# tomstrident/GAN-based-Video-Style-Transfer

Hardware: AMD Instinct MI355X
Metric: frames/sec: CycleGAN train step (G+D+flow-warp loss) 256x256 (higher is better)
Workload: dtype fp32; 1 GPU; C2: CycleGANCon optimize_parameters, resnet_9blocks G + basic PatchGAN D, ngf=ndf=64, 256x256, B_local=4, pool_size=50, flow-warp temporal loss; global_batch=4, height=256, width=256, parallelism=dp1

## Files before the change

### gan-based-video-style-transfer_amd/_lib.py

```python
import ctypes
import glob
import os
import subprocess

import torch

PKG = os.path.dirname(os.path.abspath(__file__))
REPO = os.path.dirname(PKG)
BUILD = os.path.join(PKG, "_build")
LIB_PATH = os.path.join(BUILD, "libvst_hip.so")
LIB_PATH = os.environ.get("VST_LIB_VARIANT") or LIB_PATH
CSRC = os.path.join(PKG, "csrc")
HIPCC = os.environ.get("HIPCC", "/opt/rocm/bin/hipcc")
ARCH = "gfx950"

_lib = None


def source_stamp():
    import hashlib
    h = hashlib.sha1()
    for f in sorted(glob.glob(os.path.join(CSRC, "*"))) + [os.path.join(REPO, "include", "vst_hip.h")]:
        if f.endswith((".hip", ".h")):
            h.update(os.path.basename(f).encode())
# ... 39 lines not shown
    "vst_instnorm_ws_bytes": (SZ, [I, I, I]),
    "vst_instnorm_stats": (I, [P, P, P, I, I, I, F, P]),
    "vst_instnorm_act_fwd": (I, [P, P, P, P, I, I, I, I, F, P]),
    "vst_instnorm_act_bwd": (I, [P, P, P, P, P, P, I, I, I, I, F, I, P]),
    "vst_instnorm_act_bwd_planes": (I, [P, P, P, P, P, P, I, I, I, I, F, I, P, L, P]),
    "vst_conv2d_wgrad_nhwc_ok": (I, [I, I, I, I, I, I, I, I, I, I, I, I]),
    "vst_conv2d_wgrad_nhwc_ws_bytes": (SZ, [I, I, I, I, I, I, I, I, I, I, I, I]),
    "vst_conv2d_wgrad_nhwc": (I, [P, P, P, P, SZ, I, I, I, I, I, I, I, I, I, I, I, I, I, I, L, L, I, I, P]),
    "vst_conv2d_wgrad_nhwc_f32_ok": (I, [I, I, I, I, I, I, I, I, I, I, I, I]),
    "vst_conv2d_wgrad_nhwc_f32_ws_bytes": (SZ, [I, I, I, I, I, I, I, I, I, I, I, I]),
    "vst_conv2d_wgrad_nhwc_f32": (I, [P, P, P, P, SZ, I, I, I, I, I, I, I, I, I, I, I, I, I, I, L, L, I, I, P]),
    "vst_conv2d_wgrad_pre": (I, [P, P, P, P, P, P, SZ, I, I, I, I, I, I, I, I, I, I, I, I, I, I, L, L, I, I, P]),
    "vst_instnorm_act_fwd_cp": (I, [P, P, P, P, P, I, I, I, I, I, F, I, I, I, P]),
    "vst_instnorm_act_fwd_planes": (I, [P, P, P, P, P, I, I, I, I, I, F, I, I, I, P]),
    "vst_cp_ld": (L, [L]),
    "vst_conv2d_fwd_co": (I, [P, P, P, P, P, I, I, I, I, I, I, I, I, I, I, I, F, I, I, P]),
    "vst_conv2d_fwd_co_ws_bytes": (SZ, [I, I, I, I, I, I, I, I, I, I, I]),
    "vst_conv2d_fwd_co_ws": (I, [P, P, P, P, P, I, I, I, I, I, I, I, I, I, I, I, F, I, I, P, SZ, P]),
    "vst_tapfold_planes": (I, [P, P, L, I, I, I, I, I, I, I, P]),
    "vst_conv2d_fwd_ws_bytes": (SZ, [I, I, I, I, I, I, I, I, I, I]),
    "vst_conv2d_fwd_ws": (I, [P, P, P, P, P, I, I, I, I, I, I, I, I, I, I, I, F, I, P, P, P, SZ, P]),
    "vst_c4_dgrad_frame": (I, [P, P, P, I, I, I, I, I, I, P]),
    "vst_conv_plan_fwd_tail": (I, [I, I, I, I, I, I, I, I, I, I, P]),
    "vst_act_bwd": (I, [P, P, P, L, I, F, P]),
    "vst_warp_fwd": (I, [P, P, P, I, I, I, I, I, P]),
    "vst_warp_bwd_input": (I, [P, P, P, I, I, I, I, I, P]),
    "vst_fbcheck": (I, [P, P, P, I, I, I, P]),
    "vst_loss_part_floats": (I, [L]),
    "vst_loss_temporal": (I, [P, P, P, P, P, P, I, I, I, I, I, F, P]),
    "vst_loss_temporal_bwd": (I, [P, P, P, P, P, P, P, I, I, I, I, I, F, P]),
    "vst_loss_l1": (I, [P, P, P, P, L, I, I, F, P]),
    "vst_loss_l1_bwd": (I, [P, P, P, P, L, I, I, F, P]),
    "vst_loss_mse_const": (I, [P, F, P, P, L, I, I, F, P]),
    "vst_loss_mse_const_bwd": (I, [P, F, P, P, L, I, I, F, P]),
    "vst_finish_sum": (I, [P, I, P, D, P]),
    "vst_adam_step": (I, [P, P, P, P, L, F, F, F, F, I, P]),
    "vst_axpby": (I, [P, P, L, F, F, P]),
    "vst_warp_masked_fwd": (I, [P, P, P, I, I, I, I, I, P]),
    "vst_warp_masked_bwd_input": (I, [P, P, P, I, I, I, I, I, P]),
    "vst_warp_bwd_det_ws_bytes": (SZ, [I, I, I]),
    "vst_warp_bwd_input_det": (I, [P, P, P, P, SZ, I, I, I, I, I, I, I, I, P]),
    "vst_temporal_sqdiff_part_floats": (I, [I, I, I, I]),
    "vst_temporal_sqdiff_fwd": (I, [P, P, P, P, P, P, P, P, I, I, I, I, I, F, F, P]),
    "vst_temporal_sqdiff_bwd": (I, [P, P, P, P, P, P, P, P, P, I, I, I, I, I, F, F, P]),
    "vst_resize_bilinear": (I, [P, P, P, I, I, I, I, I, I, P]),
    "vst_instnorm_affine_fwd": (I, [P, P, P, P, P, F, P, P, I, I, I, I, F, P]),
# ... 180 lines not shown
```

### gan-based-video-style-transfer_amd/csrc/common.h

```cpp
#pragma once
#include <hip/hip_runtime.h>
#include <stdint.h>
#include <stdio.h>
#include <string.h>

#include "../../include/vst_hip.h"

typedef float f32x16 __attribute__((ext_vector_type(16)));
typedef float f32x4v __attribute__((ext_vector_type(4)));

namespace vst {

void set_error(const char* fmt, ...);

inline int check_launch(const char* what) {
  hipError_t e = hipGetLastError();
  if (e != hipSuccess) {
    set_error("%s: %s", what, hipGetErrorString(e));
    return VST_EHIP;
  }
  return VST_OK;
}

#define VST_NUM_CUS 256
// ... 101 lines not shown
int bf_fprop_launch(const float* x, const void* wsplit, long wps, const float* bias, float* y, int N,
                    int H, int W, int C, int Ho, int Wo, int Cop, int R, int S, int st, int padh, int padw,
                    int reflect, int act, float slope, int math, int kind, hipStream_t s,
                    double* part = nullptr, float* tws = nullptr, size_t tws_floats = 0, const float* addend = nullptr,
                    int oph = 0);
bool tap64_ok(int Cx, int R, int W, int math);
int tap64_launch(const float* x, const void* wsplit, long wps, const float* bias, float* y, int N, int H, int W,
                 int pad, int reflect, int act, float slope, int math, hipStream_t s);
bool c4_direct_ok(int C, int Cop, int R, int S, int st, int Ho, int Wo, int math);
int c4_direct_launch(const float* x, const void* wsplit, long wps, const float* bias, float* y, int N, int H, int W,
                     int Ho, int Wo, int R, int S, int pad, int reflect, int act, float slope, int math, double* part,
                     hipStream_t s);
bool bf_dgrad_refl1_ok(int N, int H, int W, int Cy, int Cx, int math);
size_t bf_dgrad_refl1_ws_floats(int N, int H, int W, int Cy, int Cx, int math);
size_t bf_dgrad_refl1_slabs(int N, int H, int W, int Cy, int Cx, int math, BorderSlabs* b);
int bf_dgrad_refl1_launch(const float* dy, const void* wsplit, long wps, const float* addend, float* dx, int N, int H,
                          int W, int Cy, int Cx, int math, hipStream_t s, float* ws, size_t ws_floats, bool add_border);
bool bf_dgrad_refl1_inb_ok(int N, int H, int W, int Cy, int Cx, int math);
int bf_dgrad_refl1_inb_slices(int H, int W);
int bf_dgrad_refl1_inb_launch(const float* dy, const void* wsplit, long wps, const float* addend, float* dx, int N,
                              int H, int W, int Cy, int Cx, int math, hipStream_t s, float* ws, size_t ws_floats,
                              const float* z, const float* st, double* part, int act, float slope,
                              const __bf16* apl = nullptr, long pps = 0);
size_t bf_fprop_ws_floats(long M, int Cop, int C, int R, int S, int math);
int bf_tail_ks(long M, int Cop, int m_split, int nk);
void bf_split_plan(long M, int Cop, int C, int R, int S, int math, int kind, int* m_first, int* ks_out);
void bf_plan(long M, int Cop, int math, int kind, int* kind_out, int* m_split_out, int* tail_out);
void bf_nhwc_to_planes(const float* x, void* y, long P, int Cs, int np, hipStream_t s, int row_in = 0,
                       int row_out = 0);
void bf_wgrad_launch(const float* xt, const void* dyp, float* slab, int N, int H, int W, int Cx, int Ho,
                     int Wo, int Cyp, int S, int pad, int st, int Mw, int chunk, int nsplit, int kind, int math,
                     hipStream_t s);
void bf_wgrad_geom(int kind, int math, int* bm, int* bn, int* bk, int* slots);
bool bf_wgrad_nhwc_ok(int kind, int Wo, int Cx, int Cyp);
void bf_wgrad_nhwc_launch(const float* x, const void* dy, long pps, bool bf32, float* slab, int N, int H, int W,
                          int Cx, int Ho, int Wo, int Cyp, int S, int pad, int st, int reflect, int Mw, int chunk,
                          int nsplit, int kind, hipStream_t s, float* dwd = nullptr, int dco = 0, int dacc = 0);

void rk_tile_geom(int kind, int math, int* bm, int* bn, int* bk, int* slots);
void rk_nhwc_to_cp(const float* x, float* y, long P, int Cs, int pack, hipStream_t s);
void rk_nhwc_to_cp_pad(const float* x, float* y, int N, int H, int W, int Cs, int pad, int reflect,
                       int phase, int pack, hipStream_t s, int extra = 0);
void rk_wgrad_launch(const float* xt, const float* dyt, float* slab, int N, int H, int W, int Cx,
                     int Ho, int Wo, int Cyp, int S, int pad, int st, int Mw, int chunk,
                     int nsplit, int kind, int math, hipStream_t s);
void rk_tconv_launch(const float* in, const float* wp, const float* bias, const float* addend,
// ... 29 lines not shown
```

### gan-based-video-style-transfer_amd/csrc/conv.hip

```cpp
#include "common.h"

namespace vst {

constexpr int BK = 32;

template <int BM, int BN, int WM, int WN>
struct Tile {
  static constexpr int NW = (BM / WM) * (BN / WN);
  static constexpr int NT = 64 * NW;
  static constexpr int LDA = BM + 4;
  static constexpr int LDB = BN + 4;
  static constexpr int WAVES_N = BN / WN;
  static constexpr int MI = WM / 32;
  static constexpr int NI = WN / 32;
  static constexpr int A_ELEMS = BK * LDA;
  static constexpr int B_ELEMS = BK * LDB;
  static constexpr int STAGE = A_ELEMS + B_ELEMS;
  static_assert(NW == 4 || NW == 8, "4 or 8 waves per block");
  static_assert(WM % 32 == 0 && WN % 32 == 0, "32x32 MFMA blocks");
};

template <int BM, int BN, int WM, int WN, class Hook>
__device__ __forceinline__ void mma_stage(const float* __restrict__ As, const float* __restrict__ Bs,
                                          f32x16 (&acc)[WM / 32][WN / 32], int wm0, int wn0, int lane,
// ... 867 lines not shown
  return bf_fprop_ws_floats((long)N * Ho * Wo, Cop, Cx, R, S, math) * sizeof(float);
}

extern "C" int vst_conv2d_fwd_ws(const float* x, const float* wp, const void* wsplit, const float* bias, float* y,
                                 int N, int H, int W, int Cx, int Cop, int R, int S, int stride, int pad, int pad_mode,
                                 int act, float slope, int math, double* part, int* nsplit, float* ws,
                                 size_t ws_bytes, void* stream) {
  return conv_fwd_impl(x, wp, wsplit, bias, y, N, H, W, Cx, Cop, R, S, stride, pad, pad, pad_mode, act, slope,
                       math, (hipStream_t)stream, part, nsplit, ws, ws_bytes);
}

extern "C" int vst_conv_plan_fwd_tail(int N, int H, int W, int Cx, int Cop, int R, int S, int stride, int pad,
                                      int math, int* ksplit) {
  VST_REQUIRE(ksplit, "conv_plan_fwd_tail: null");
  *ksplit = 0;
  const size_t b = vst_conv2d_fwd_ws_bytes(N, H, W, Cx, Cop, R, S, stride, pad, math);
  if (b) {
    const int Ho = (H + 2 * pad - R) / stride + 1, Wo = (W + 2 * pad - S) / stride + 1;
    int mf;
    bf_split_plan((long)N * Ho * Wo, Cop, Cx, R, S, math, -1, &mf, ksplit);
  }
  return VST_OK;
}

extern "C" int vst_conv2d_fwd_hwp(const float* x, const float* wp, const void* wsplit, const float* bias, float* y,
                                  int N, int H, int W, int Cx, int Cop, int R, int S, int stride, int pad_h, int pad_w,
                                  int pad_mode, int act, float slope, int math, void* stream) {
  return conv_fwd_impl(x, wp, wsplit, bias, y, N, H, W, Cx, Cop, R, S, stride, pad_h, pad_w, pad_mode, act, slope,
                       math, (hipStream_t)stream);
}

extern "C" int vst_conv2d_fwd_hw(const float* x, const float* wp, const void* wsplit, const float* bias,
                                 float* y, int N, int H, int W, int Cx, int Cop, int R, int S, int stride,
                                 int pad_h, int pad_w, int act, float slope, int math, void* stream) {
  return conv_fwd_impl(x, wp, wsplit, bias, y, N, H, W, Cx, Cop, R, S, stride, pad_h, pad_w, VST_PAD_ZERO, act,
                       slope, math, (hipStream_t)stream);
}

extern "C" size_t vst_conv2d_fwd_hw_ws_bytes(int N, int H, int W, int Cx, int Cop, int R, int S, int stride, int pad_h,
                                             int pad_w, int math) {
  if (N <= 0 || H <= 0 || W <= 0 || R <= 0 || S <= 0 || stride <= 0 || Cx % 8 || Cop == 4) return 0;
  const int Ho = (H + 2 * pad_h - R) / stride + 1, Wo = (W + 2 * pad_w - S) / stride + 1;
  if (Ho <= 0 || Wo <= 0 || g_tile_override[0] >= 0) return 0;
  return bf_fprop_ws_floats((long)N * Ho * Wo, Cop, Cx, R, S, math) * sizeof(float);
}

// ... 472 lines not shown
```

### gan-based-video-style-transfer_amd/csrc/conv_bf.hip

```cpp
#include <type_traits>

#include "common.h"

#ifndef VST_BF_X6K3
#define VST_BF_X6K3 0
#endif
#ifndef VST_BF_MINB
#define VST_BF_MINB 1
#endif
#ifndef VST_BF_X6_256
#define VST_BF_X6_256 1
#endif
#ifndef VST_BF_KSLICE
#define VST_BF_KSLICE 1
#endif
#ifndef VST_BF_TAIL_KIND
#define VST_BF_TAIL_KIND 8
#endif
#ifndef VST_BF_TAIL
#define VST_BF_TAIL 1
#endif
#ifndef VST_BF_SCHED
#define VST_BF_SCHED 1
#endif
#ifndef VST_BF_PRIO
// ... 390 lines not shown
    if (!SA) {
      prep(P ^ 1);
      store_stage<T>(nxt, ra[P ^ 1], rbv[P ^ 1], rb, kq, !dmab.active, !dmab.a_active);
    }
    mma16<T>(mid, hi, acc);
    mma16<T>(hi, mid, acc);
    if (VST_M16_SCHED) sched16<2 * NM, RA ? 0 : NR, 0, SA ? 0 : 2, SA ? 0 : NW>();
    __builtin_amdgcn_sched_barrier(0);
    __syncthreads();
    read_plane16<T>(mid, nxt, 1, wm0, wn0, lane);
    mma16<T>(hi, hi, acc);
    mma16<T>(lo, hi, acc);
    mma16<T>(hi, lo, acc);
    if (VST_M16_SCHED) sched16<3 * NM, NR, 0, 0, 0>();
  };
  int kt = 0;
  for (; kt + 1 < nk; kt += 2) {
    step(kt, std::integral_constant<int, 0>());
    step(kt + 1, std::integral_constant<int, 1>());
  }
  if (kt < nk) step(kt, std::integral_constant<int, 0>());
}

template <int MI, int NI>
__device__ __forceinline__ void zero_acc4(f32x4v (&acc)[MI][NI]) {
#pragma unroll
  for (int i = 0; i < MI; ++i)
#pragma unroll
    for (int j = 0; j < NI; ++j) acc[i][j] = f32x4v{0.f, 0.f, 0.f, 0.f};
}

template <int MI, int NI>
__device__ __forceinline__ void zero_acc(f32x16 (&acc)[MI][NI]) {
#pragma unroll
  for (int i = 0; i < MI; ++i)
#pragma unroll
    for (int j = 0; j < NI; ++j)
#pragma unroll
      for (int r = 0; r < 16; ++r) acc[i][j][r] = 0.f;
}

__device__ __forceinline__ int remap_mtile(int bx, int nx) {
  if ((nx & 7) != 0) return bx;
  return (bx & 7) * (nx >> 3) + (bx >> 3);
}

// ... 204 lines not shown
  __syncthreads();
  if (t < 192) {
    const int v = t >> 6, cc = t & 63, nn = blockIdx.z * 64 + cc;
    if (nn >= C) return;
    double acc = 0.0;
    if (v < 2)
      for (int q = 0; q < 16; ++q) acc += red[v][q][cc];
    inb.part[(((long)n * inb.ns + first_slice + blockIdx.x) * C + nn) * 3 + v] = acc;
  }
}

__device__ __forceinline__ int phase_row(int mm, int oph, int Ho, int Wo) {
  const bool full = oph > 4;
  const int q = full ? oph - 5 : oph - 1, a = q >> 1, b = q & 1;
  const int hw = Ho * Wo, n = mm / hw, rem = mm - n * hw, ph = rem / Wo, pw = rem - ph * Wo;
  const int H = full ? Ho - 1 : Ho - a, W = full ? Wo - 1 : Wo - b;
  const int i = ph - a, j = pw - b;
  if (i < 0 || j < 0 || i >= H || j >= W) return -1;
  return (n * 2 * H + 2 * i + a) * 2 * W + 2 * j + b;
}

__device__ __attribute__((aligned(256))) float g_zero_page[64];

template <class T, bool KSL, int REFL, bool SPLIT, bool APRE = false>
__device__ __forceinline__ void conv_fprop_bf_body(
    int bid, const float* __restrict__ x, const __bf16* __restrict__ ws, long wps, const float* __restrict__ bias,
    float* __restrict__ y, int H, int W, int C, int Ho, int Wo, int Cop, int S, int st, int padh,
    int padw, int reflect, int act, float slope, int M, int Ktot, int m_base, double* __restrict__ part,
    int spk, float* __restrict__ slab, const float* __restrict__ addend, int oph,
    InbArgs inb = InbArgs{}, const __bf16* __restrict__ apl = nullptr, long pps = 0) {
  static_assert(!SPLIT || KSL, "split-K needs the channel-slice-major K walk");
  static_assert(REFL < 4 || (SPLIT && KSL), "border rows run as split-K slabs");
  __shared__ __attribute__((aligned(16))) char smem[2 * T::STAGE];
  constexpr int A_LD = T::A_LD, B_LD = T::B_LD, RPP = T::RPP, NP = T::NP;
  const int t = threadIdx.x, lane = t & 63, wave = t >> 6;
  int mt_, nt_;
  const int Mt_ = (M - m_base + T::BM - 1) / T::BM, Nt_ = (Cop + T::BN - 1) / T::BN;
  const int zs = SPLIT ? bid / (Mt_ * Nt_) : 0;
  tile_of(SPLIT ? bid - zs * Mt_ * Nt_ : bid, Mt_, Nt_, mt_, nt_);
  const int m0 = m_base + mt_ * T::BM, n0 = nt_ * T::BN;
  const int kq = t % T::KC, rb = t / T::KC;
  const float* zp = g_zero_page;

  constexpr bool C4 = REFL == 3;
  const int seg = REFL != 5 ? 0 : (m0 < Ho ? 0 : (m0 < 2 * Ho ? 1 : (m0 < 2 * Ho + Wo ? 2 : 3)));
  const int Sx = REFL != 5 ? S : (seg < 2 ? 3 : 1);
  int hb[A_LD], wb[A_LD], pb[A_LD], aoff[A_LD], aoff2[C4 ? A_LD : 1];
#pragma unroll
  for (int j = 0; j < A_LD; ++j) {
    const int m = m0 + rb + RPP * j;
    const int mm = m < M ? m : 0;
    if constexpr (REFL == 5) {
      const int L = seg < 2 ? W + 2 : H;
      const int r = mm - (seg == 0 ? 0 : (seg == 1 ? Ho : (seg == 2 ? 2 * Ho : 2 * Ho + Wo)));
      const int n = r / L, k = r - n * L;
      const bool live = (unsigned)r < (unsigned)(st * L);
// ... 184 lines not shown
      ts = go ? (w1 ? 0 : ts1) : ts;
      tr = go ? (w2 ? 0 : tr1) : tr;
      ksb = go ? ksb + (w2 ? T::BK : 0) : ksb;
      tap_rows(tr, ts);
      return;
    }
    if (!go) return;
    kcur += T::BK;
    kc += T::BK;
    if (kc >= C) {
      do {
        kc -= C;
        if (++ks == S) { ks = 0; ++kr; }
      } while (kc >= C);
      tap_rows(kr, ks);
    }
  };

  auto prep = [](int) __attribute__((always_inline)) {};
  const int wm0 = (wave / T::WAVES_N) * T::WM, wn0 = (wave % T::WAVES_N) * T::WN;
  if constexpr (T::M16) {
    f32x4v acc[T::MI16][T::NI16];
    zero_acc4(acc);
    if constexpr (GLDS)
      main_loop16<T>(smem, nk, acc, ra, rbv, rb, kq, load_all, adv, prep, DmaB<decltype(dma_b), GLDS_A>{dma_b});
    else
      main_loop16<T>(smem, nk, acc, ra, rbv, rb, kq, load_all, adv, prep, NoDma{});
    if constexpr (SPLIT) {
      float* sl = slab + (long)zs * (M - m_base) * Cop;
#pragma unroll
      for (int i = 0; i < T::MI16; ++i)
#pragma unroll
        for (int j = 0; j < T::NI16; ++j) {
          const int n = n0 + wn0 + 16 * j + (lane & 15);
#pragma unroll
          for (int r = 0; r < 4; ++r) {
            const int mm = m0 + wm0 + 16 * i + 4 * (lane >> 4) + r;
            if (n < Cop && mm < M) sl[(long)(mm - m_base) * Cop + n] = acc[i][j][r];
          }
        }
      return;
    }
    constexpr bool LFIT = T::BM * (T::BN + 16) * 4 <= 2 * T::STAGE;
    const bool LEPI = LFIT && (VST_BF_LDS_EPI || addend != nullptr || oph != 0 || inb.part != nullptr);
    constexpr int LDE = T::BN + 16;
    float* ept = reinterpret_cast<float*>(smem);
    constexpr int IC4 = T::BN / 4, IRW = 64 / (IC4 > 0 ? IC4 : 1);
// ... 160 lines not shown
        s1 += __shfl_xor(s1, 32);
        s2 += __shfl_xor(s2, 32);
        const int g0 = m0 + wm0 + 32 * i;
        if (lane < 32 && nok && g0 < M) {
          const int hw = Ho * Wo, img = g0 / hw, z = (g0 - img * hw) >> 5;
          double* d = part + (((long)img * (hw >> 5) + z) * Cop + n) * 2;
          d[0] = s1;
          d[1] = s2;
        }
      }
    }
}

template <class T, bool KSL, int REFL, bool SPLIT = false, bool APRE = false>
__global__ __launch_bounds__(T::NT, T::MINB) void conv_fprop_bf_k(
    const float* __restrict__ x, const __bf16* __restrict__ ws, long wps, const float* __restrict__ bias,
    float* __restrict__ y, int H, int W, int C, int Ho, int Wo, int Cop, int S, int st, int padh,
    int padw, int reflect, int act, float slope, int M, int Ktot, int m_base, double* __restrict__ part,
    int spk = 0, float* __restrict__ slab = nullptr, const float* __restrict__ addend = nullptr, int oph = 0,
    const __bf16* __restrict__ apl = nullptr, long pps = 0) {
  conv_fprop_bf_body<T, KSL, REFL, SPLIT, APRE>(blockIdx.x, x, ws, wps, bias, y, H, W, C, Ho, Wo, Cop, S, st, padh,
                                                padw, reflect, act, slope, M, Ktot, m_base, part, spk, slab, addend, oph,
                                                InbArgs{}, apl, pps);
}

template <class T, bool APRE = false>
__global__ __launch_bounds__(T::NT, T::MINB) void conv_fprop_bf_inb_k(
    const float* __restrict__ x, const __bf16* __restrict__ ws, long wps, float* __restrict__ y, int H, int W, int C,
    int Cop, const float* __restrict__ addend, int M, int Ktot, InbArgs inb, const __bf16* __restrict__ apl = nullptr,
    long pps = 0) {
  conv_fprop_bf_body<T, true, 0, false, APRE>(blockIdx.x, x, ws, wps, nullptr, y, H, W, C, H, W, Cop, 3, 1, 1, 1, 0,
                                              VST_ACT_NONE, 0.f, M, Ktot, 0, nullptr, 0, nullptr, addend, 0, inb, apl, pps);
}

struct PhaseJobs {
  const __bf16* ws[4];
  int t0[5];
};

template <class T>
__global__ __launch_bounds__(T::NT, T::MINB) void conv_convT_phases_k(const float* __restrict__ x, PhaseJobs jobs,
                                                                      const float* __restrict__ bias,
                                                                      float* __restrict__ y, int N, int H, int W,
                                                                      int C, int Cop, int act, float slope,
                                                                      int full) {
  const int bid = blockIdx.x;
// ... 720 lines not shown
  const long b256 = ((M + 255) / 256) * ((Cop + 127) / 128);
  if (kd == 7 || b256 > VST_BF_FULLSPLIT_MAX) return;
  int bm, bn, sl;
  bf_geom(kd, 3, &bm, &bn, &sl);
  const long blocks = ((M + bm - 1) / bm) * ((Cop + bn - 1) / bn);
  const long rounds_small = (blocks + (long)sl * VST_NUM_CUS - 1) / ((long)sl * VST_NUM_CUS);
  const double t_small = (kd == 0 || kd == 2 || kd == 4 || kd == 9) ? 1.5 : (kd == 3 ? 1.8 : 1.2);
  const double small_us = rounds_small * nk * t_small + 3.0;
  double best = 0.85 * small_us;
  int bk = 0;
  for (int ks = 2; ks <= 32; ++ks) {
    const int steps = (nk + ks - 1) / ks;
    if (steps < 4 || (long)(ks - 1) * steps >= nk) continue;
    const long rounds = (b256 * ks + VST_NUM_CUS - 1) / VST_NUM_CUS;
    const double us = rounds * (steps * 2.25 + 4.0) + (double)(ks + 1) * M * Cop * 4.0 / 4.0e6 + 3.0;
    if (us < best) {
      best = us;
      bk = ks;
    }
  }
  *ks_out = bk;
}

size_t bf_fprop_ws_floats(long M, int Cop, int C, int R, int S, int math) {
  int mf, ks;
  bf_split_plan(M, Cop, C, R, S, math, -1, &mf, &ks);
  return ks ? (size_t)ks * (M - mf) * Cop : 0;
}

int bf_fprop_launch(const float* x, const void* wsplit, long wps, const float* bias, float* y, int N,
                    int H, int W, int C, int Ho, int Wo, int Cop, int R, int S, int st, int padh, int padw,
                    int reflect, int act, float slope, int math, int kind, hipStream_t s, double* part,
                    float* tws, size_t tws_floats, const float* addend, int oph) {
  if (oph) tws = nullptr;
  VST_REQUIRE(!(part && addend), "conv fprop: IN partials together with an addend are not supported");
  const int M = N * Ho * Wo, K = R * S * C;
  if (kind < 0 && padh == padw && !addend && !oph && c4_direct_ok(C, Cop, R, S, st, Ho, Wo, math))
    return c4_direct_launch(x, wsplit, wps, bias, y, N, H, W, Ho, Wo, R, S, padh, reflect, act, slope, math, part, s);
  const __bf16* ws = reinterpret_cast<const __bf16*>(wsplit);
  int kd, m_split, tail_kind;
  bf_plan(M, Cop, math, kind, &kd, &m_split, &tail_kind);
  int ks = 0, m_first = 0;
  if (tws) {
    bf_split_plan(M, Cop, C, R, S, math, kind, &m_first, &ks);
    if ((size_t)ks * (M - m_first) * Cop > tws_floats) ks = 0;
    if (ks && !m_first) {
// ... 19 lines not shown
                         nullptr, addend, oph);                                                          \
    else                                                                                            \
      hipLaunchKernelGGL((bf::conv_fprop_bf_k<T, false, 2>), grid, dim3(T::NT), 0, s, x, ws, wps, bias, y, \
                         H, W, C, Ho, Wo, Cop, S, st, padh, padw, reflect, act, slope, Mend, K, mb, part, 0,      \
                         nullptr, addend, oph);                                                          \
  }
  for (int ph = (ks && !m_first) ? 1 : 0; ph < ((m_split || (ks && !m_first)) ? 2 : 1); ++ph) {
    const int mb = ph ? m_split : 0, Mend = (m_split && !ph) ? m_split : M;
    const int kp = ph ? tail_kind : kd;
    if (ph == 1 && ks) {
      using T = bf::Tile<256, 128, 64, 64, 32, 3>;
      const int nk = (K + T::BK - 1) / T::BK, spk = (nk + ks - 1) / ks;
      const dim3 grid(ceil_div(M - mb, 256) * ceil_div(Cop, 128) * ks);
      if (reflect)
        hipLaunchKernelGGL((bf::conv_fprop_bf_k<T, true, 1, true>), grid, dim3(T::NT), 0, s, x, ws, wps, bias, y, H,
                           W, C, Ho, Wo, Cop, S, st, padh, padw, reflect, act, slope, M, K, mb, part, spk, tws,
                           nullptr);
      else
        hipLaunchKernelGGL((bf::conv_fprop_bf_k<T, true, 0, true>), grid, dim3(T::NT), 0, s, x, ws, wps, bias, y, H,
                           W, C, Ho, Wo, Cop, S, st, padh, padw, reflect, act, slope, M, K, mb, part, spk, tws,
                           nullptr);
      hipLaunchKernelGGL(bf::fprop_splitk_reduce_k, dim3(ceil_div(M - mb, 32), ceil_div(Cop, 64)), dim3(256), 0, s,
                         tws, ks, mb, M, Cop, bias, act, slope, y, part, Ho * Wo, addend);
      continue;
    }
    if (math == VST_MATH_BF16X6) {
      VST_BF_DISPATCH(kp, 3, VST_BF)
    } else {
      VST_BF_DISPATCH(kp, 2, VST_BF)
    }
  }
#undef VST_BF
  return check_launch("conv2d_fwd(bf16 split)");
}


static void bf_border_plan(int N, int H, int W, int Cy, int Cx, int math, int* ks_out, long* mb_out) {
  const int NB = bf::dgrad_border_rows(H, W);
  const long Mb = (long)N * NB;
  const int bm = math == VST_MATH_BF16X6 ? 256 : 128;
  const long tiles = ((Mb + bm - 1) / bm) * ((Cx + 127) / 128);
  const int nk = (9 * Cy + 31) / 32;
  int ks = (int)(VST_NUM_CUS / (tiles > 0 ? tiles : 1));
  ks = ks < 1 ? 1 : (ks > 16 ? 16 : ks);
  while (ks > 1 && (ks - 1) * ((nk + ks - 1) / ks) >= nk) --ks;
  *ks_out = ks;
// ... 332 lines not shown
```

### gan-based-video-style-transfer_amd/ops.py

```python
import os
import threading

import torch

from . import _lib

ACT = {"none": 0, "relu": 1, "lrelu": 2, "tanh": 3}
PAD = {"zero": 0, "reflect": 1}
PACK_KC, PACK_CK, PACK_OK, PACK_IK, PACK_IKF, PACK_SOK = 0, 1, 2, 3, 4, 5
PACK_FWD, PACK_DGRAD = PACK_OK, PACK_IK
EUNSUPPORTED = 2
IN_EPS = 1e-5


def cpad(c):
    return (c + 3) // 4 * 4


def lib():
    return _lib.load()


def _stream():
    return torch.cuda.current_stream().cuda_stream
# ... 136 lines not shown
            return p, ev
    return None


def _probe_end(h):
    if h is not None:
        p, ev = h
        ev[1].record()
        p.events.append(ev)


FWD_SPLITK = True

_plan_memo = {}
_tiles = threading.local()


def _memo(plan, *inputs):
    key = (plan.__name__, inputs, getattr(_tiles, "v", None))
    r = _plan_memo.get(key)
    if r is None:
        r = _plan_memo[key] = plan(*inputs)
    return r


def _fwd_ws(N, H, W, Cx, cop, R, S, stride, pad, m, device):
    nb = _memo(lib().vst_conv2d_fwd_ws_bytes, N, H, W, Cx, cop, R, S, stride, pad, m) if FWD_SPLITK else 0
    if nb == 0:
        return None, 0
    return torch.empty((nb + 3) // 4, device=device), nb


def conv2d_fwd(x, wp, bias, cop, R, S, stride, pad, pad_mode="zero", act="none", slope=0.0,
               out=None, role="fwd", co_real=None):
    _dev_check(x, wp, bias)
    if co_real is not None and co_real < cop:
        N, H, W, Cx = x.shape
        Ho = (H + 2 * pad - R) // stride + 1
        Wo = (W + 2 * pad - S) // stride + 1
        y = out if out is not None else torch.empty((N, Ho, Wo, cop), device=x.device)
        nb = int(lib().vst_conv2d_fwd_co_ws_bytes(N, H, W, Cx, cop, R, S, stride, pad, PAD[pad_mode], int(co_real)))
        ws = torch.empty((nb + 3) // 4, device=x.device) if nb else None
        _call("vst_conv2d_fwd_co_ws", _p(x), _p(wp), _p(getattr(wp, "vst_split", None)), _p(bias), _p(y), N, H, W,
              Cx, cop, R, S, stride, pad, PAD[pad_mode], ACT[act], float(slope), _math(role), int(co_real), _p(ws), nb,
              _stream())
        return y
    N, H, W, Cx = x.shape
    Ho = (H + 2 * pad - R) // stride + 1
    Wo = (W + 2 * pad - S) // stride + 1
    y = out if out is not None else torch.empty((N, Ho, Wo, cop), device=x.device)
    m = _math(role)
    ws, nb = _fwd_ws(N, H, W, Cx, cop, R, S, stride, pad, m, x.device) if S == R else (None, 0)
    h = _probe_begin("fwd", (N, H, W, Cx, cop, R, stride, pad, pad_mode)) if _probes else None
    if ws is not None:
        _call("vst_conv2d_fwd_ws", _p(x), _p(wp), _p(getattr(wp, "vst_split", None)), _p(bias), _p(y), N, H, W, Cx,
              cop, R, S, stride, pad, PAD[pad_mode], ACT[act], float(slope), m, None, None, _p(ws), nb, _stream())
    else:
        _call("vst_conv2d_fwd", _p(x), _p(wp), _p(getattr(wp, "vst_split", None)), _p(bias), _p(y), N, H,
              W, Cx, cop, R, S, stride, pad,
              PAD[pad_mode], ACT[act], float(slope), m, _stream())
    _probe_end(h)
    return y


def conv2d_fwd_in(x, wp, bias, cop, R, S, stride, pad, pad_mode="zero", role="fwd"):
    import ctypes
    _dev_check(x, wp, bias)
    N, H, W, Cx = x.shape
    Ho = (H + 2 * pad - R) // stride + 1
    Wo = (W + 2 * pad - S) // stride + 1
    y = torch.empty((N, Ho, Wo, cop), device=x.device)
    hw = Ho * Wo
    part = torch.empty((N * max(1, hw // 32) * cop * 2,), device=x.device, dtype=torch.float64)
    nsplit = ctypes.c_int(0)
    m = _math(role)
    ws, nb = _fwd_ws(N, H, W, Cx, cop, R, S, stride, pad, m, x.device) if S == R else (None, 0)
    h = _probe_begin("fwd", (N, H, W, Cx, cop, R, stride, pad, pad_mode)) if _probes else None
    _call("vst_conv2d_fwd_ws", _p(x), _p(wp), _p(getattr(wp, "vst_split", None)), _p(bias), _p(y), N, H, W, Cx,
          cop, R, S, stride, pad, PAD[pad_mode], ACT["none"], 0.0, m, _p(part),
          ctypes.addressof(nsplit), _p(ws), nb, _stream())
    _probe_end(h)
    if nsplit.value == 0:
        return y, instnorm_stats(y)
    stats = torch.empty((N, cop, 2), device=x.device)
    _call("vst_instnorm_finalize", _p(part), _p(stats), N, hw, cop, nsplit.value, IN_EPS, _stream())
    return y, stats


def conv2d_tfwd(x, wp, bias, Ho, Wo, cx, R, S, stride, pad, act="none", slope=0.0,
                pad_mode="zero", addend=None, role="bwd", co_real=None):
    _dev_check(x, wp, bias, addend)
    N, Hi, Wi, Cy = x.shape
    y = torch.empty((N, Ho, Wo, cx), device=x.device)
    if co_real is not None and co_real < Cy:
        _call("vst_conv2d_tfwd_co", _p(x), _p(wp), _p(bias), _p(addend), _p(y), N, Hi, Wi, Cy, Ho, Wo, cx,
              R, S, stride, pad, PAD[pad_mode], ACT[act], float(slope), _math(role), int(co_real), _stream())
        return y
    _call("vst_conv2d_tfwd", _p(x), _p(wp), _p(bias), _p(addend), _p(y), N, Hi, Wi, Cy, Ho, Wo, cx,
          R, S, stride, pad, PAD[pad_mode], ACT[act], float(slope), _math(role), _stream())
    return y
# ... 1050 lines not shown
    _dev_check(x, bias)
    N, H, W, Cx = x.shape
    m = _math(role)
    if CONVT_DIRECT and m != _lib.MATH_MODES["fp32"] and Cx % 8 == 0 and cop != 4 and \
            all(getattr(wp, "vst_split", None) is not None for wp in packs):
        y = torch.empty((N, 2 * H, 2 * W, cop), device=x.device)
        if CONVT_GROUPED and Cx % 32 == 0:
            _call("vst_conv2d_convT_s2", _p(x), *[_p(wp.vst_split) for wp in packs], _p(bias), _p(y), N, H, W, Cx,
                  cop, ACT[act], 0.0, m, _stream())
            return y
        for (a, b), wp in zip(((0, 0), (0, 1), (1, 0), (1, 1)), packs):
            _call("vst_conv2d_fwd_phase", _p(x), _p(wp.vst_split), _p(bias), _p(y), N, H, W, Cx, cop, a, b, ACT[act],
                  0.0, m, _stream())
        return y
    outs = []
    for (a, b), wp in zip(((0, 0), (0, 1), (1, 0), (1, 1)), packs):
        outs.append(conv2d_fwd_hw(x, wp, bias, cop, 1 + a, 1 + b, 1, a, b, act=act, role=role))
    y = torch.empty((N, 2 * H, 2 * W, cop), device=x.device)
    _call("vst_interleave_phases", _p(outs[0]), _p(outs[1]), _p(outs[2]), _p(outs[3]), _p(y), N, H, W, cop,
          _stream())
    return y


_ROUTE_FLAGS = ("FWD_SPLITK", "FWD_HW_SPLITK", "DGRAD_BORDER", "C4_DGRAD", "TAP_CHUNK_BYTES", "TAP_PLANES", "TAP_SWAP",
                "C4S2_GROUPED", "CONVT_DIRECT", "CONVT_GROUPED")
_NET_ROUTE_FLAGS = ("C8_EDGES", "C4_FWD", "DGRAD_AS_FPROP", "TAP_LAST", "TAP_H", "CONVT_PHASES", "IN_XT", "D_CO1")


def route_flags():
    import sys
    g = globals()
    net = sys.modules.get(__name__.rsplit(".", 1)[0] + ".networks")
    return tuple(g[n] for n in _ROUTE_FLAGS) + (tuple(getattr(net, n) for n in _NET_ROUTE_FLAGS) if net else ())


_lib.apply_route_overrides(__name__, globals())
```

### include/vst_hip.h

```cpp
#ifndef VST_HIP_H
#define VST_HIP_H

#include <stddef.h>
#include <stdint.h>

#ifdef __cplusplus
extern "C" {
#endif

enum { VST_OK = 0, VST_EINVAL = 1, VST_EUNSUPPORTED = 2, VST_EHIP = 3 };
enum { VST_PAD_ZERO = 0, VST_PAD_REFLECT = 1 };
enum { VST_ACT_NONE = 0, VST_ACT_RELU = 1, VST_ACT_LRELU = 2, VST_ACT_TANH = 3 };
enum { VST_PACK_KC = 0,
       VST_PACK_CK = 1,
       VST_PACK_OK = 2,
       VST_PACK_IK = 3,
       VST_PACK_IKF = 4,
       VST_PACK_SOK = 5 };

const char* vst_last_error(void);
int vst_version(void);
const char* vst_build_info(void);

int vst_nchw_to_nhwc(const float* x, float* y, int N, int C, int H, int W, int Cs, void* stream);
int vst_nhwc_to_nchw(const float* x, float* y, int N, int C, int H, int W, int Cs, void* stream);
int vst_weight_pack(const float* w, float* out, int O, int I, int R, int S, int Op, int Ip,
                    int mode, void* stream);
int vst_weight_split(const float* w, void* out, long n, void* stream);
int vst_weight_pack_split(const float* w, float* out, void* split, int O, int I, int R, int S, int Op, int Ip,
                          int mode, void* stream);
int vst_weight_pack_batch(const void* jobs, int njobs, long nblocks, void* stream);

enum { VST_MATH_F32 = 0, VST_MATH_BF16X3 = 1, VST_MATH_BF16X6 = 2 };
int vst_conv2d_fwd(const float* x, const float* wp, const void* wsplit, const float* bias, float* y,
                   int N, int H, int W, int Cx, int Cop, int R, int S, int stride, int pad,
                   int pad_mode, int act, float slope, int math, void* stream);
size_t vst_conv2d_fwd_ws_bytes(int N, int H, int W, int Cx, int Cop, int R, int S, int stride, int pad,
                               int math);
int vst_conv2d_fwd_ws(const float* x, const float* wp, const void* wsplit, const float* bias, float* y, int N,
                      int H, int W, int Cx, int Cop, int R, int S, int stride, int pad, int pad_mode, int act,
                      float slope, int math, double* part, int* nsplit, float* ws, size_t ws_bytes, void* stream);
int vst_c4_dgrad_frame(const float* dy, const float* w, float* dx, int N, int H, int W, int C, int R, int pad,
                       void* stream);
int vst_conv_plan_fwd_tail(int N, int H, int W, int Cx, int Cop, int R, int S, int stride, int pad, int math,
                           int* ksplit);
int vst_conv2d_fwd_co(const float* x, const float* wp, const void* wsplit, const float* bias, float* y, int N, int H,
                      int W, int Cx, int Cop, int R, int S, int stride, int pad, int pad_mode, int act, float slope,
                      int math, int co_real, void* stream);
size_t vst_conv2d_fwd_co_ws_bytes(int N, int H, int W, int Cx, int Cop, int R, int S, int stride, int pad,
                                  int pad_mode, int co_real);
int vst_conv2d_fwd_co_ws(const float* x, const float* wp, const void* wsplit, const float* bias, float* y, int N,
                         int H, int W, int Cx, int Cop, int R, int S, int stride, int pad, int pad_mode, int act,
                         float slope, int math, int co_real, float* ws, size_t ws_bytes, void* stream);
int vst_conv2d_fwd_in(const float* x, const float* wp, const void* wsplit, const float* bias, float* y, int N,
                      int H, int W, int Cx, int Cop, int R, int S, int stride, int pad, int pad_mode, int act,
                      float slope, int math, double* part, int* nsplit, void* stream);
int vst_conv2d_tfwd(const float* in, const float* wp, const float* bias, const float* addend,
                    float* out, int N, int Hi, int Wi, int Cy, int Ho, int Wo, int Cx, int R,
                    int S, int stride, int pad, int pad_mode, int act, float slope, int math,
                    void* stream);
int vst_conv2d_tfwd_co(const float* in, const float* wp, const float* bias, const float* addend, float* out, int N,
                       int Hi, int Wi, int Cy, int Ho, int Wo, int Cx, int R, int S, int stride, int pad, int pad_mode,
                       int act, float slope, int math, int co_real, void* stream);
size_t vst_conv2d_wgrad_ws_bytes(int N, int H, int W, int Cx, int Ho, int Wo, int Cyp, int R, int S,
                                 int stride);
int vst_conv2d_wgrad(const float* x, const float* dy, float* dw, float* ws, size_t ws_bytes, int N,
                     int H, int W, int Cx, int Ho, int Wo, int Cyp, int R, int S, int stride,
                     int pad, int pad_mode, int Co, int Ci, long so, long si, int accumulate,
// ... 283 lines not shown
```

Measured before the change: 79.18 frames/s.

## Add halo-patch forward conv kernel reusing shared input tile across 3x3 taps

Adds a forward 3x3 stride-1 reflect-pad conv path for the bf16x6 math mode that loads a spatial input patch plus halo into LDS once per K-slice. All nine taps then read from that patch by shifting addresses, instead of re-gathering im2col rows for each tap. The goal is to cut global/LDS load traffic for the resnet-block convs (W=64 or 32). It enlarges LDS use and adds a routing flag, which is on by default, plus a planning query. The risk is lower occupancy and more complex synchronisation in the new main loop.

```diff
diff --git a/gan-based-video-style-transfer_amd/_lib.py b/gan-based-video-style-transfer_amd/_lib.py
--- a/gan-based-video-style-transfer_amd/_lib.py
+++ b/gan-based-video-style-transfer_amd/_lib.py
@@ -85,6 +85,8 @@
     "vst_conv2d_fwd_ws": (I, [P, P, P, P, P, I, I, I, I, I, I, I, I, I, I, I, F, I, P, P, P, SZ, P]),
     "vst_c4_dgrad_frame": (I, [P, P, P, I, I, I, I, I, I, P]),
     "vst_conv_plan_fwd_tail": (I, [I, I, I, I, I, I, I, I, I, I, P]),
+    "vst_conv_plan_fwd_halo": (I, [I, I, I, I, I, I, I, I, I, I, I, I, P]),
+    "vst_route_fwd_halo": (None, [I]),
     "vst_act_bwd": (I, [P, P, P, L, I, F, P]),
     "vst_warp_fwd": (I, [P, P, P, I, I, I, I, I, P]),
     "vst_warp_bwd_input": (I, [P, P, P, I, I, I, I, I, P]),
diff --git a/gan-based-video-style-transfer_amd/csrc/common.h b/gan-based-video-style-transfer_amd/csrc/common.h
--- a/gan-based-video-style-transfer_amd/csrc/common.h
+++ b/gan-based-video-style-transfer_amd/csrc/common.h
@@ -147,6 +147,9 @@
                               int H, int W, int Cy, int Cx, int math, hipStream_t s, float* ws, size_t ws_floats,
                               const float* z, const float* st, double* part, int act, float slope,
                               const __bf16* apl = nullptr, long pps = 0);
+void bf_set_fwd_halo(int on);
+long bf_halo_plan_rows(long M, int H, int W, int C, int Cop, int Ho, int Wo, int R, int S, int st, int padh, int padw,
+                       int reflect, int math, int kind, bool splitk);
 size_t bf_fprop_ws_floats(long M, int Cop, int C, int R, int S, int math);
 int bf_tail_ks(long M, int Cop, int m_split, int nk);
 void bf_split_plan(long M, int Cop, int C, int R, int S, int math, int kind, int* m_first, int* ks_out);
diff --git a/gan-based-video-style-transfer_amd/csrc/conv.hip b/gan-based-video-style-transfer_amd/csrc/conv.hip
--- a/gan-based-video-style-transfer_amd/csrc/conv.hip
+++ b/gan-based-video-style-transfer_amd/csrc/conv.hip
@@ -913,6 +913,19 @@
   }
   return VST_OK;
 }
+
+extern "C" int vst_conv_plan_fwd_halo(int N, int H, int W, int Cx, int Cop, int R, int S, int stride, int pad,
+                                      int pad_mode, int math, int splitk, long* rows) {
+  VST_REQUIRE(rows && N > 0 && H > 0 && W > 0 && R > 0 && S > 0 && stride > 0 && pad >= 0, "conv_plan_fwd_halo: bad args");
+  *rows = 0;
+  const int Ho = (H + 2 * pad - R) / stride + 1, Wo = (W + 2 * pad - S) / stride + 1;
+  if (Ho <= 0 || Wo <= 0 || Cx % 8) return VST_OK;
+  *rows = bf_halo_plan_rows((long)N * Ho * Wo, H, W, Cx, Cop, Ho, Wo, R, S, stride, pad, pad,
+                            pad_mode == VST_PAD_REFLECT, math, g_tile_override[0], splitk && g_tile_override[0] < 0);
+  return VST_OK;
+}
+
+extern "C" void vst_route_fwd_halo(int on) { bf_set_fwd_halo(on); }
 
 extern "C" int vst_conv2d_fwd_hwp(const float* x, const float* wp, const void* wsplit, const float* bias, float* y,
                                   int N, int H, int W, int Cx, int Cop, int R, int S, int stride, int pad_h, int pad_w,
diff --git a/gan-based-video-style-transfer_amd/csrc/conv_bf.hip b/gan-based-video-style-transfer_amd/csrc/conv_bf.hip
--- a/gan-based-video-style-transfer_amd/csrc/conv_bf.hip
+++ b/gan-based-video-style-transfer_amd/csrc/conv_bf.hip
@@ -1,6 +1,8 @@
+#include <atomic>
 #include <type_traits>
 
 #include "common.h"
+#include "halo_geom.h"
 
 #ifndef VST_BF_X6K3
 #define VST_BF_X6K3 0
@@ -437,6 +439,89 @@
   if (kt < nk) step(kt, std::integral_constant<int, 0>());
 }
 
+template <class T, int WT, class LoadPatch, class StorePatch, class Adv, class DmaB>
+__device__ __forceinline__ void halo_loop16(char* smem, int nk, f32x4v (&acc)[T::MI16][T::NI16], LoadPatch load_patch,
+                                            StorePatch store_patch, Adv adv, DmaB dma_b) {
+  constexpr int PW = halo::patch_pitch(WT), PLA = halo::patch_slots(WT) * halo::kSlotBytes;
+  constexpr int BST = T::NP * T::B_PLANE;
+  static_assert(T::BM == halo::kTileM && T::M16 && T::WM == 64 && (WT == 32 || WT == 64), "halo: the 256-row x6 M16 tile");
+  const int t = threadIdx.x, lane = t & 63, wave = t >> 6;
+  const int wm0 = (wave / T::WAVES_N) * T::WM, wn0 = (wave % T::WAVES_N) * T::WN;
+  const int li = lane & 15, c = lane >> 4;
+  if (nk <= 0) return;
+  char* const bs0 = smem + 3 * PLA;
+  constexpr int NA = 64 / WT, FA = T::MI16 / NA;
+  const int abase = halo::tap_slot(WT, wm0 / WT, li, 0, 0);
+  int ao[NA];
+  const int boff = swz_off<T>(wn0 + li, c);
+  static_assert(T::SWS == 2 && T::KC == 4, "halo: B rows 16 apart share their chunk keying");
+  auto tap_addr = [&](int toff) __attribute__((always_inline)) {
+#pragma unroll
+    for (int a = 0; a < NA; ++a) ao[a] = halo::chunk_off(abase + a * PW + toff, c);
+  };
+  auto read_ab = [&](Plane16<T>& f, int p, const char* bs) __attribute__((always_inline)) {
+#pragma unroll
+    for (int i = 0; i < T::MI16; ++i)
+      f.a[i] = *reinterpret_cast<const bf16x8_t*>(smem + p * PLA + ao[i / FA] + (i % FA) * 16 * halo::kSlotBytes);
+#pragma unroll
+    for (int j = 0; j < T::NI16; ++j)
+      f.b[j] = *reinterpret_cast<const bf16x8_t*>(bs + p * T::B_PLANE + boff + j * 16 * T::ROWB);
+  };
+  dma_b(bs0);
+  load_patch();
+  __syncthreads();
+  store_patch();
+  adv(nk > 1);
+  tap_addr(0);
+  __syncthreads();
+  Plane16<T> hi, mid, lo;
+  read_ab(mid, 1, bs0);
+  load_patch();
+  int cr = 0, cs = 0;
+  auto step = [&](int kt, auto par) __attribute__((always_inline)) {
+    constexpr int P = decltype(par)::value;
+    const char* cur = bs0 + P * BST;
+    char* nxt = bs0 + (P ^ 1) * BST;
+    dma_b(nxt);
+    adv(kt + 2 < nk);
+    read_ab(hi, 0, cur);
+    mma16<T>(mid, mid, acc);
+    read_ab(lo, 2, cur);
+    mma16<T>(mid, hi, acc);
+    mma16<T>(hi, mid, acc);
+    const bool last = cr == 2 && cs == 2;
+    const bool w1 = cs == 2;
+    cs = w1 ? 0 : cs + 1;
+    cr = last ? 0 : (w1 ? cr + 1 : cr);
+    __builtin_amdgcn_sched_barrier(0);
+    if (last && kt + 1 < nk) {
+      __syncthreads();
+      store_patch();
+      tap_addr(0);
+      mma16<T>(hi, hi, acc);
+      mma16<T>(lo, hi, acc);
+      mma16<T>(hi, lo, acc);
+      __builtin_amdgcn_sched_barrier(0);
+      __syncthreads();
+      read_ab(mid, 1, nxt);
+      load_patch();
+    } else {
+      tap_addr(cr * PW + cs);
+      __syncthreads();
+      read_ab(mid, 1, nxt);
+      mma16<T>(hi, hi, acc);
+      mma16<T>(lo, hi, acc);
+      mma16<T>(hi, lo, acc);
+    }
+  };
+  int kt = 0;
+  for (; kt + 1 < nk; kt += 2) {
+    step(kt, std::integral_constant<int, 0>());
+    step(kt + 1, std::integral_constant<int, 1>());
+  }
+  if (kt < nk) step(kt, std::integral_constant<int, 0>());
+}
+
 template <int MI, int NI>
 __device__ __forceinline__ void zero_acc4(f32x4v (&acc)[MI][NI]) {
 #pragma unroll
@@ -687,7 +772,7 @@
 
 __device__ __attribute__((aligned(256))) float g_zero_page[64];
 
-template <class T, bool KSL, int REFL, bool SPLIT, bool APRE = false>
+template <class T, bool KSL, int REFL, bool SPLIT, bool APRE = false, int HALO = 0>
 __device__ __forceinline__ void conv_fprop_bf_body(
     int bid, const float* __restrict__ x, const __bf16* __restrict__ ws, long wps, const float* __restrict__ bias,
     float* __restrict__ y, int H, int W, int C, int Ho, int Wo, int Cop, int S, int st, int padh,
@@ -696,7 +781,8 @@
     InbArgs inb = InbArgs{}, const __bf16* __restrict__ apl = nullptr, long pps = 0) {
   static_assert(!SPLIT || KSL, "split-K needs the channel-slice-major K walk");
   static_assert(REFL < 4 || (SPLIT && KSL), "border rows run as split-K slabs");
-  __shared__ __attribute__((aligned(16))) char smem[2 * T::STAGE];
+  constexpr int HALO_LDS = halo::lds_bytes(HALO != 0 ? HALO : 64);
+  __shared__ __attribute__((aligned(16))) char smem[HALO != 0 && HALO_LDS > 2 * T::STAGE ? HALO_LDS : 2 * T::STAGE];
   constexpr int A_LD = T::A_LD, B_LD = T::B_LD, RPP = T::RPP, NP = T::NP;
   const int t = threadIdx.x, lane = t & 63, wave = t >> 6;
   int mt_, nt_;
@@ -927,7 +1013,85 @@
   if constexpr (T::M16) {
     f32x4v acc[T::MI16][T::NI16];
     zero_acc4(acc);
-    if constexpr (GLDS)
+    if constexpr (HALO != 0) {
+      static_assert(GLDS && !APRE && !SPLIT && REFL <= 1 && B_LD == 1, "halo: fp32 x, whole K, zero / reflect pad 1");
+      constexpr int NS = halo::patch_slots(HALO), PLA = NS * halo::kSlotBytes;
+      constexpr int NREG = halo::kRegSlots, NSTG = NS - NREG, NPC = halo::stage_pieces(HALO);
+      constexpr int STG = 3 * PLA + 2 * NP * T::B_PLANE;
+      static_assert(NREG == T::NT / 4 && NSTG > 0 && STG + NPC * 1024 == halo::lds_bytes(HALO), "halo: staging area");
+      const int hw = H * W, img = m0 / hw, h0 = (m0 - img * hw) / HALO;
+      auto slot_off = [&](int slot) __attribute__((always_inline)) {
+        const int src = halo::slot_src(slot < NS ? slot : NS - 1, h0, H, HALO, REFL == 1);
+        return src < 0 ? -1 : (img * hw + src) * C;
+      };
+      const int wave_u = __builtin_amdgcn_readfirstlane(wave);
+      float4 pr[2];
+      int pks = 0;
+      auto load_patch = [&]() __attribute__((always_inline)) {
+        {
+          const int o = slot_off(t >> 2);
+          const float* p = o >= 0 ? x + o + pks + 8 * (t & 3) : zp;
+          pr[0] = *reinterpret_cast<const float4*>(p);
+          pr[1] = *reinterpret_cast<const float4*>(p + 4);
+        }
+#pragma unroll
+        for (int k = 0; k < (NPC + T::NW - 1) / T::NW; ++k) {
+          const int q = wave_u + T::NW * k;
+          if (q < NPC) {
+            const int o = slot_off(NREG + 8 * q + (lane >> 3));
+            const float* p = o >= 0 ? x + o + pks + 4 * (lane & 7) : zp;
+#if defined(__HIP_DEVICE_COMPILE__)
+            __builtin_amdgcn_global_load_lds(p, (lds_void*)(smem + STG + q * 1024), 16, 0, 0);
+#endif
+          }
+        }
+        pks = pks + T::BK < C ? pks + T::BK : pks;
+      };
+      auto store_patch = [&]() __attribute__((always_inline)) {
+        {
+          uint4 s[NP];
+          split8<NP>(pr[0], pr[1], s);
+          const int off = halo::chunk_off(t >> 2, t & 3);
+#pragma unroll
+          for (int p = 0; p < NP; ++p) *reinterpret_cast<uint4*>(smem + p * PLA + off) = s[p];
+        }
+#pragma unroll
+        for (int k = 0; k < (4 * NSTG + T::NT - 1) / T::NT; ++k) {
+          const int e = t + T::NT * k;
+          if (e < 4 * NSTG) {
+            const float4* raw = reinterpret_cast<const float4*>(smem + STG + e * 32);
+            uint4 s[NP];
+            split8<NP>(raw[0], raw[1], s);
+            const int off = halo::chunk_off(NREG + (e >> 2), e & 3);
+#pragma unroll
+            for (int p = 0; p < NP; ++p) *reinterpret_cast<uint4*>(smem + p * PLA + off) = s[p];
+          }
+        }
+      };
+      auto adv_b = [&](bool go) __attribute__((always_inline)) {
+        const int ts1 = ts + 1;
+        const bool w1 = ts1 == 3;
+        const int tr1 = tr + (w1 ? 1 : 0);
+        const bool w2 = w1 && tr1 == 3;
+        ts = go ? (w1 ? 0 : ts1) : ts;
+        tr = go ? (w2 ? 0 : tr1) : tr;
+        ksb = go ? ksb + (w2 ? T::BK : 0) : ksb;
+      };
+      const int nrow = n0 + rb < Cop ? n0 + rb : Cop - 1;
+      const unsigned blane = (unsigned)nrow * (unsigned)Ktot + 8u * (unsigned)((t % T::KC) ^ T::swz(rb));
+      const int brow0 = __builtin_amdgcn_readfirstlane(rb - (lane / T::KC));
+      auto dma_bh = [&](char* bs) __attribute__((always_inline)) {
+        const __bf16* base = ws + ((tr * 3 + ts) * C + ksb);
+#pragma unroll
+        for (int p = 0; p < NP; ++p) {
+#if defined(__HIP_DEVICE_COMPILE__)
+          __builtin_amdgcn_global_load_lds(base + p * wps + blane, (lds_void*)(bs + p * T::B_PLANE + brow0 * T::ROWB), 16, 0,
+                                           0);
+#endif
+        }
+      };
+      halo_loop16<T, HALO>(smem, nk, acc, load_patch, store_patch, adv_b, dma_bh);
+    } else if constexpr (GLDS)
       main_loop16<T>(smem, nk, acc, ra, rbv, rb, kq, load_all, adv, prep, DmaB<decltype(dma_b), GLDS_A>{dma_b});
     else
       main_loop16<T>(smem, nk, acc, ra, rbv, rb, kq, load_all, adv, prep, NoDma{});
@@ -1134,6 +1298,15 @@
   conv_fprop_bf_body<T, KSL, REFL, SPLIT, APRE>(blockIdx.x, x, ws, wps, bias, y, H, W, C, Ho, Wo, Cop, S, st, padh,
                                                 padw, reflect, act, slope, M, Ktot, m_base, part, spk, slab, addend, oph,
                                                 InbArgs{}, apl, pps);
+}
+
+template <class T, int REFL, int HALO>
+__global__ __launch_bounds__(T::NT, T::MINB) void conv_fprop_bf_halo_k(
+    const float* __restrict__ x, const __bf16* __restrict__ ws, long wps, const float* __restrict__ bias,
+    float* __restrict__ y, int H, int W, int C, int Cop, int act, float slope, int M, int Ktot, int m_base,
+    double* __restrict__ part, const float* __restrict__ addend) {
+  conv_fprop_bf_body<T, true, REFL, false, false, HALO>(blockIdx.x, x, ws, wps, bias, y, H, W, C, H, W, Cop, 3, 1, 1, 1,
+                                                        REFL, act, slope, M, Ktot, m_base, part, 0, nullptr, addend, 0);
 }
 
 template <class T, bool APRE = false>
@@ -1900,6 +2073,27 @@
   *ks_out = bk;
 }
 
+static std::atomic<int> g_fwd_halo{1};
+void bf_set_fwd_halo(int on) { g_fwd_halo.store(on ? 1 : 0); }
+
+bool bf_halo_ok(int H, int W, int C, int Ho, int Wo, int R, int S, int st, int padh, int padw, int reflect, int math,
+                int kp, long mb, long Mend) {
+  return VST_BF_GLDS_B && VST_BF_MF16 && VST_BF_KSLICE && math == VST_MATH_BF16X6 && kp == 7 && padh == padw && reflect &&
+         halo::shape_ok(H, W, C, R, S, st, padh) && Ho == H && Wo == W && mb % halo::kTileM == 0 && Mend > mb &&
+         (Mend - mb) % halo::kTileM == 0;
+}
+
+long bf_halo_plan_rows(long M, int H, int W, int C, int Cop, int Ho, int Wo, int R, int S, int st, int padh, int padw,
+                       int reflect, int math, int kind, bool splitk) {
+  if (C == 4 || Cop == 4 || math != VST_MATH_BF16X6) return 0;
+  int kd, m_split, tail_kind, ks = 0, m_first = 0;
+  bf_plan(M, Cop, math, kind, &kd, &m_split, &tail_kind);
+  if (splitk) bf_split_plan(M, Cop, C, R, S, math, kind, &m_first, &ks);
+  if (ks && !m_first) return 0;
+  const long rows = m_split ? m_split : M;
+  return bf_halo_ok(H, W, C, Ho, Wo, R, S, st, padh, padw, reflect, math, kd, 0, rows) ? rows : 0;
+}
+
 size_t bf_fprop_ws_floats(long M, int Cop, int C, int R, int S, int math) {
   int mf, ks;
   bf_split_plan(M, Cop, C, R, S, math, -1, &mf, &ks);
@@ -1965,6 +2159,17 @@
                            nullptr);
       hipLaunchKernelGGL(bf::fprop_splitk_reduce_k, dim3(ceil_div(M - mb, 32), ceil_div(Cop, 64)), dim3(256), 0, s,
                          tws, ks, mb, M, Cop, bias, act, slope, y, part, Ho * Wo, addend);
+      continue;
+    }
+    if (g_fwd_halo.load() && !oph && bf_halo_ok(H, W, C, Ho, Wo, R, S, st, padh, padw, reflect, math, kp, mb, Mend)) {
+      using T = bf::Tile<256, 128, 64, 64, 32, 3>;
+      const dim3 grid((Mend - mb) / 256 * ceil_div(Cop, 128));
+      if (W == 64)
+        hipLaunchKernelGGL((bf::conv_fprop_bf_halo_k<T, 1, 64>), grid, dim3(T::NT), 0, s, x, ws, wps, bias, y, H, W, C,
+                           Cop, act, slope, Mend, K, mb, part, addend);
+      else
+        hipLaunchKernelGGL((bf::conv_fprop_bf_halo_k<T, 1, 32>), grid, dim3(T::NT), 0, s, x, ws, wps, bias, y, H, W, C,
+                           Cop, act, slope, Mend, K, mb, part, addend);
       continue;
     }
     if (math == VST_MATH_BF16X6) {
diff --git a/gan-based-video-style-transfer_amd/csrc/halo_geom.h b/gan-based-video-style-transfer_amd/csrc/halo_geom.h
--- /dev/null
+++ b/gan-based-video-style-transfer_amd/csrc/halo_geom.h
@@ -0,0 +1,50 @@
+#pragma once
+
+#if defined(__HIPCC__) || defined(__CUDACC__)
+#define VST_HALO_HD __host__ __device__ constexpr
+#else
+#define VST_HALO_HD constexpr
+#endif
+
+namespace vst {
+namespace halo {
+
+constexpr int kTileM = 256;
+constexpr int kSlotBytes = 64;
+constexpr int kMaxLds = 160 * 1024;
+constexpr int kRegSlots = 128;
+
+VST_HALO_HD int tile_rows(int W) { return kTileM / W; }
+VST_HALO_HD int patch_rows(int W) { return kTileM / W + 2; }
+VST_HALO_HD int patch_pitch(int W) { return W + 2; }
+VST_HALO_HD int patch_slots(int W) { return patch_rows(W) * patch_pitch(W); }
+VST_HALO_HD int stage_pieces(int W) { return (patch_slots(W) - kRegSlots + 7) / 8; }
+VST_HALO_HD int lds_bytes(int W) {
+  return 3 * patch_slots(W) * kSlotBytes + 2 * 3 * 128 * 64 + stage_pieces(W) * 1024;
+}
+
+VST_HALO_HD bool shape_ok(int H, int W, int C, int R, int S, int stride, int pad) {
+  return R == 3 && S == 3 && stride == 1 && pad == 1 && (W == 32 || W == 64) && H >= 2 && C > 0 && C % 32 == 0 &&
+         (H * W) % kTileM == 0 && lds_bytes(W) <= kMaxLds;
+}
+
+VST_HALO_HD int tap_slot(int W, int lr, int wo, int r, int s) { return (lr + r) * patch_pitch(W) + wo + s; }
+
+VST_HALO_HD int reflect(int i, int n) { return i < 0 ? -i : (i >= n ? 2 * n - 2 - i : i); }
+
+VST_HALO_HD int slot_src(int slot, int h0, int H, int W, bool refl) {
+  const int pw = patch_pitch(W), pr = slot / pw, pc = slot - pr * pw;
+  int h = h0 - 1 + pr, w = pc - 1;
+  if (refl) {
+    h = reflect(h, H);
+    w = reflect(w, W);
+  } else if (h < 0 || h >= H || w < 0 || w >= W) {
+    return -1;
+  }
+  return h * W + w;
+}
+
+VST_HALO_HD int chunk_off(int p, int c) { return (p << 6) | ((c << 4) ^ ((p << 3) & 32)); }
+
+}
+}
diff --git a/gan-based-video-style-transfer_amd/ops.py b/gan-based-video-style-transfer_amd/ops.py
--- a/gan-based-video-style-transfer_amd/ops.py
+++ b/gan-based-video-style-transfer_amd/ops.py
@@ -182,6 +182,30 @@
     if r is None:
         r = _plan_memo[key] = plan(*inputs)
     return r
+
+
+FWD_HALO = True
+_halo_sent = None
+
+
+def _sync_halo():
+    global _halo_sent
+    if _halo_sent is not FWD_HALO:
+        lib().vst_route_fwd_halo(1 if FWD_HALO else 0)
+        _halo_sent = FWD_HALO
+
+
+def conv_plan_fwd_halo(N, H, W, Cx, Cop, R, S, stride, pad, pad_mode="reflect", math="fwd"):
+    return _memo(_halo_plan, N, H, W, Cx, Cop, R, S, stride, pad, PAD[pad_mode], _math(math), FWD_SPLITK) \
+        if FWD_HALO else 0
+
+
+def _halo_plan(N, H, W, Cx, Cop, R, S, stride, pad, pm, m, splitk):
+    import ctypes
+    rows = ctypes.c_long(0)
+    _call("vst_conv_plan_fwd_halo", N, H, W, Cx, Cop, R, S, stride, pad, pm, m, 1 if (splitk and R == S) else 0,
+          ctypes.addressof(rows))
+    return rows.value
 
 
 def _fwd_ws(N, H, W, Cx, cop, R, S, stride, pad, m, device):
@@ -212,6 +236,7 @@
     m = _math(role)
     ws, nb = _fwd_ws(N, H, W, Cx, cop, R, S, stride, pad, m, x.device) if S == R else (None, 0)
     h = _probe_begin("fwd", (N, H, W, Cx, cop, R, stride, pad, pad_mode)) if _probes else None
+    _sync_halo()
     if ws is not None:
         _call("vst_conv2d_fwd_ws", _p(x), _p(wp), _p(getattr(wp, "vst_split", None)), _p(bias), _p(y), N, H, W, Cx,
               cop, R, S, stride, pad, PAD[pad_mode], ACT[act], float(slope), m, None, None, _p(ws), nb, _stream())
@@ -236,6 +261,7 @@
     m = _math(role)
     ws, nb = _fwd_ws(N, H, W, Cx, cop, R, S, stride, pad, m, x.device) if S == R else (None, 0)
     h = _probe_begin("fwd", (N, H, W, Cx, cop, R, stride, pad, pad_mode)) if _probes else None
+    _sync_halo()
     _call("vst_conv2d_fwd_ws", _p(x), _p(wp), _p(getattr(wp, "vst_split", None)), _p(bias), _p(y), N, H, W, Cx,
           cop, R, S, stride, pad, PAD[pad_mode], ACT["none"], 0.0, m, _p(part),
           ctypes.addressof(nsplit), _p(ws), nb, _stream())
@@ -1332,7 +1358,7 @@
     return y
 
 
-_ROUTE_FLAGS = ("FWD_SPLITK", "FWD_HW_SPLITK", "DGRAD_BORDER", "C4_DGRAD", "TAP_CHUNK_BYTES", "TAP_PLANES", "TAP_SWAP",
+_ROUTE_FLAGS = ("FWD_SPLITK", "FWD_HALO", "FWD_HW_SPLITK", "DGRAD_BORDER", "C4_DGRAD", "TAP_CHUNK_BYTES", "TAP_PLANES", "TAP_SWAP",
                 "C4S2_GROUPED", "CONVT_DIRECT", "CONVT_GROUPED")
 _NET_ROUTE_FLAGS = ("C8_EDGES", "C4_FWD", "DGRAD_AS_FPROP", "TAP_LAST", "TAP_H", "CONVT_PHASES", "IN_XT", "D_CO1")
 
diff --git a/include/vst_hip.h b/include/vst_hip.h
--- a/include/vst_hip.h
+++ b/include/vst_hip.h
@@ -44,6 +44,9 @@
                        void* stream);
 int vst_conv_plan_fwd_tail(int N, int H, int W, int Cx, int Cop, int R, int S, int stride, int pad, int math,
                            int* ksplit);
+int vst_conv_plan_fwd_halo(int N, int H, int W, int Cx, int Cop, int R, int S, int stride, int pad, int pad_mode,
+                           int math, int splitk, long* rows);
+void vst_route_fwd_halo(int on);
 int vst_conv2d_fwd_co(const float* x, const float* wp, const void* wsplit, const float* bias, float* y, int N, int H,
                       int W, int Cx, int Cop, int R, int S, int stride, int pad, int pad_mode, int act, float slope,
                       int math, int co_real, void* stream);
```

Measured after the change: 79.82 frames/s, median of 6. Within noise of the previous version (+0.8%).
